# cvg/pixel-perfect-sfm

Measured on AMD Instinct MI355X. Metric: featuremetric residuals+Jacobians evaluated/sec (1M obs), higher is better.
Workload: dtype f32 horizontal / f64 vertical+normalisation on f16 patches; 1 GPU; BASELINE.json configs[2]: synthetic 200 cams / 200000 points / 1000000 obs featuremetric BA residual+Jacobian evaluation, 128-ch fp16 16x16 patches, SIMPLE_RADIAL, fused six-scalar Jacobian reduction; n_obs=1000000, channels=128, patch=16, obs_per_gpu=1000000, partition=none

## Files before the change

pixel-perfect-sfm_amd/csrc/pxr_ba_solve.hip:

```cpp
#include <hip/hip_runtime.h>

#include <algorithm>
#include <chrono>
#include <cmath>
#include <cstdlib>
#include <cstring>
#include <limits>
#include <thread>
#include <vector>

#include "pxr_ba_pcg.h"
#include "pxr_ba_solve.h"
#include "pxr_device.h"
#include "pxr_internal.h"

namespace pxr {


constexpr int JAC_THREADS = 128;

__global__ __launch_bounds__(JAC_THREADS) void k_jac(const SolveDev d, const double* __restrict__ rec,
                                                     pxr_loss loss, double* __restrict__ L, double* __restrict__ W) {
  extern __shared__ double jstage[];
  const int lane = threadIdx.x & 63, wave = threadIdx.x >> 6;
// ... 219 lines not shown
      double tr = 0.0;
      for (int x = 0; x < NP; ++x) tr += red[x];
      chunk_trace[blockIdx.x] = tr;
    }
  }
  if (sl == 0 && kpart) {
    kpart[(size_t)blockIdx.x * ne_max + e] = acc;
  } else if (sl == 0) {
    const int ra = col_index(d, img, cam, a);
    const double v = fixed ? __longlong_as_double(qacc) : acc;
    if (is_g) accum_flush(gc + ra, v, det_scale);
    else if (block_form) {
      double* Ub = U + (size_t)img * d.DC * d.DC;
      accum_flush(Ub + a * d.DC + b, v, det_scale);
      if (a != b) accum_flush(Ub + b * d.DC + a, v, det_scale);
    } else accum_flush(U + (size_t)ra * d.n_c + col_index(d, img, cam, b), v, det_scale);
  }
}

__global__ __launch_bounds__(256) void k_pinv(int64_t n_points, const int* __restrict__ pt_var,
                                              const double* __restrict__ V,
                                              const double* __restrict__ Vdiag0 ,
                                              double inv_radius, double* __restrict__ T,
                                              double* __restrict__ zero_ptr, int zero_n) {
  if (blockIdx.x == 0) for (int e = threadIdx.x; e < zero_n; e += blockDim.x) zero_ptr[e] = 0.0;
  const int64_t p = (int64_t)blockIdx.x * blockDim.x + threadIdx.x;
  if (p >= n_points) return;
  double* To = T + 6 * p;
  if (!pt_var[p]) { for (int j = 0; j < 6; ++j) To[j] = 0.0; return; }
  const double a00 = V[6 * p] + Vdiag0[3 * p] * inv_radius, a01 = V[6 * p + 1], a02 = V[6 * p + 2];
  const double a11 = V[6 * p + 3] + Vdiag0[3 * p + 1] * inv_radius, a12 = V[6 * p + 4];
  const double a22 = V[6 * p + 5] + Vdiag0[3 * p + 2] * inv_radius;
  const double c00 = a11 * a22 - a12 * a12, c01 = a02 * a12 - a01 * a22, c02 = a01 * a12 - a02 * a11;
  const double det = a00 * c00 + a01 * c01 + a02 * c02;
  const double id = 1.0 / det;
  To[0] = c00 * id; To[1] = c01 * id; To[2] = c02 * id;
  To[3] = (a00 * a22 - a02 * a02) * id; To[4] = (a01 * a02 - a00 * a12) * id;
  To[5] = (a00 * a11 - a01 * a01) * id;
}

struct Copy4 { const double* src[4]; double* dst[4]; int64_t n[4]; };
__global__ __launch_bounds__(256) void k_copy4(const Copy4 c) {
  const int64_t stride = (int64_t)gridDim.x * blockDim.x, t0 = (int64_t)blockIdx.x * blockDim.x + threadIdx.x;
#pragma unroll
  for (int a = 0; a < 4; ++a)
    for (int64_t e = t0; e < c.n[a]; e += stride) c.dst[a][e] = c.src[a][e];
}

__global__ __launch_bounds__(256) void k_schur(const SolveDev d, const int64_t* __restrict__ pt_ptr,
                                               const int64_t* __restrict__ pt_obs,
                                               const double* __restrict__ W, const double* __restrict__ T,
                                               const double* __restrict__ gp, double* __restrict__ S,
                                               double* __restrict__ rhs, double det_scale) {
  const int64_t tid = (int64_t)blockIdx.x * blockDim.x + threadIdx.x;
  const int64_t i = tid / d.DC;
  const int a = (int)(tid - i * d.DC);
  if (i >= d.v.n_obs) return;
  const int img = d.v.d_obs_image[i], cam = d.v.d_image_camera[img];
  const int dci = d.pose_dim[img] + d.intr_dim[cam];
  if (a >= dci) return;
  const int pt = d.v.d_obs_point[i];
  if (!d.pt_var[pt]) return;
  double y0, y1, y2;
  y_row(W, T, i, a, d.DC, pt, y0, y1, y2);
  const int r = col_index(d, img, cam, a);
  accum_add(rhs + (size_t)r * d.ldS, -(y0 * gp[3 * (size_t)pt] + y1 * gp[3 * (size_t)pt + 1] + y2 * gp[3 * (size_t)pt + 2]), det_scale);
  for (int64_t o = pt_ptr[pt]; o < pt_ptr[pt + 1]; ++o) {
    const int64_t j = pt_obs[o];
    const int imgj = d.v.d_obs_image[j], camj = d.v.d_image_camera[imgj];
// ... 82 lines not shown
            const int c = col[u];
            if (c >= 0 && c >= rrow[a])
              accum_add(acc + (size_t)a * CT + (c - c0), -(ya0 * mm[u][0] + ya1 * mm[u][1] + ya2 * mm[u][2]), det_scale);
          }
        }
      }
    }
    o = o_next; s = s_next;
  }
  __syncthreads();
  for (int e = threadIdx.x; e < dci * CT; e += blockDim.x) {
    const int a = e / CT, cl = e % CT;
    const double v = acc[(size_t)a * CT + cl];
    if (__double_as_longlong(v) != 0ll) accum_flush(S + (size_t)col_index(d, img, cam, a) * d.ldS + (c0 + cl), v, det_scale);
  }
  if (blockIdx.y == 0 && threadIdx.x < dci) {
    const double v = racc[threadIdx.x];
    if (__double_as_longlong(v) != 0ll) accum_flush(rhs + (size_t)col_index(d, img, cam, threadIdx.x) * d.ldS, v, det_scale);
  }
}

__global__ void k_copy_upper_add_diag(int n, const double* __restrict__ U, const double* __restrict__ damp,
                                      double inv_radius, const double* __restrict__ gc, double* __restrict__ S,
                                      int add_u, double det_scale) {
  const int64_t t = (int64_t)blockIdx.x * blockDim.x + threadIdx.x;
  const int ld = n + 1;
  if (t >= (int64_t)n * ld) return;
  const int r = (int)(t / ld), c = (int)(t % ld);
  double v = S[t];
  if (add_u) {
    v = (c < n && r <= c) ? U[(size_t)r * n + c] : 0.0;
  }
  else {
    if (det_scale != 0.0) v = (double)__double_as_longlong(v) / det_scale;
    if (r == c) v += damp[r] * inv_radius;
    if (c == n) v += gc[r];
  }
  S[t] = v;
}

__global__ void k_extract_diag(int n, const double* __restrict__ U, double* __restrict__ out) {
  const int i = blockIdx.x * blockDim.x + threadIdx.x;
  if (i < n) out[i] = U[(size_t)i * n + i];
}

__global__ void k_clamp(int64_t n, const double* __restrict__ in, double lo, double hi, double* __restrict__ out) {
  const int64_t i = (int64_t)blockIdx.x * blockDim.x + threadIdx.x;
  if (i < n) out[i] = fmin(fmax(in[i], lo), hi);
}

__global__ void k_point_diag(int64_t n_points, const double* __restrict__ V, double* __restrict__ out) {
  const int64_t p = (int64_t)blockIdx.x * blockDim.x + threadIdx.x;
  if (p >= n_points) return;
  out[3 * p] = V[6 * p]; out[3 * p + 1] = V[6 * p + 3]; out[3 * p + 2] = V[6 * p + 5];
}

__global__ void k_jacobi_scale(int64_t n, const double* __restrict__ diag, double* __restrict__ scale) {
  const int64_t i = (int64_t)blockIdx.x * blockDim.x + threadIdx.x;
  if (i < n) scale[i] = 1.0 / (1.0 + sqrt(diag[i]));
}

__global__ void k_axpy1(int n, const double* __restrict__ x, double* __restrict__ y) {
  const int i = blockIdx.x * blockDim.x + threadIdx.x;
  if (i < n) y[i] += x[i];
}

__global__ void k_fill(int64_t n, double v, double* __restrict__ out) {
  const int64_t i = (int64_t)blockIdx.x * blockDim.x + threadIdx.x;
  if (i < n) out[i] = v;
}

__global__ void k_finish_camera_step(int n, const double* __restrict__ x, const double* __restrict__ gc,
                                     const double* __restrict__ damp, double inv_radius,
                                     double* __restrict__ delta_c, double* __restrict__ scal_rep, long long* __restrict__ limb) {
  __shared__ long long lsh[PXR_LIMBS * 4];
  const int i = blockIdx.x * blockDim.x + threadIdx.x;
  double part = 0.0;
  if (i < n) {
    const double dl = -x[i];
    delta_c[i] = dl;
    part = dl * (damp[i] * inv_radius * dl - gc[i]);
  }
  if (limb) {
    Limbs l;
    if (i < n) l.add(part);
    limbs_block_add(l, limb + (8 + 0) * PXR_LIMBS, lsh);
    return;
  }
  for (int off = 32; off > 0; off >>= 1) part += __shfl_xor(part, off);
  if ((threadIdx.x & 63) == 0) atomicAdd(scal_rep + 0, part);
}

constexpr int BACKSUB_PPG = 8;
template <int G>
__global__ __launch_bounds__(256) void k_backsub(const SolveDev d, const int64_t* __restrict__ pt_ptr,
                                                 const int* __restrict__ pj, const int4* __restrict__ pcols,
                                                 const double* __restrict__ W, const double* __restrict__ T,
                                                 const double* __restrict__ gp, const double* __restrict__ delta_c,
                                                 const double* __restrict__ Vdiag0, double inv_radius,
                                                 double* __restrict__ delta_p, double* __restrict__ scal_sum, long long* __restrict__ limb) {
  __shared__ double red[256 / 64];
  __shared__ long long lsh[PXR_LIMBS * 4];
  const int lane_a = threadIdx.x % G;
  double part = 0.0;
  Limbs lpart;
  for (int rep = 0; rep < BACKSUB_PPG; ++rep) {
  const int64_t p = ((int64_t)blockIdx.x * BACKSUB_PPG + rep) * (256 / G) + threadIdx.x / G;
  const bool live = p < d.v.n_points;
  const bool var = live && d.pt_var[p];
  double v0 = 0.0, v1 = 0.0, v2 = 0.0;
  if (var) {
    const int64_t o_end = pt_ptr[p + 1];
    for (int64_t o = pt_ptr[p]; o < o_end; o += 4) {
      int4 ci[4];
      int jj[4];
#pragma unroll
      for (int u = 0; u < 4; ++u) { const int64_t idx = min(o + u, o_end - 1); ci[u] = pcols[idx]; jj[u] = pj[idx]; }
      double w[4][3], dcv[4];
      bool ok[4];
#pragma unroll
      for (int u = 0; u < 4; ++u) {
        ok[u] = o + u < o_end && lane_a < ci[u].y + ci[u].w;
        const double* Wi = W + ((size_t)jj[u] * d.DC + (ok[u] ? lane_a : 0)) * 3;
        w[u][0] = Wi[0]; w[u][1] = Wi[1]; w[u][2] = Wi[2];
        dcv[u] = delta_c[ok[u] ? (lane_a < ci[u].y ? ci[u].x + lane_a : ci[u].z + (lane_a - ci[u].y)) : 0];
      }
#pragma unroll
      for (int u = 0; u < 4; ++u)
        if (ok[u]) { v0 += w[u][0] * dcv[u]; v1 += w[u][1] * dcv[u]; v2 += w[u][2] * dcv[u]; }
    }
  }
#pragma unroll
  for (int off = G / 2; off > 0; off >>= 1) {
    v0 += __shfl_xor(v0, off); v1 += __shfl_xor(v1, off); v2 += __shfl_xor(v2, off);
  }
  if (live && lane_a == 0) {
    double dl[3] = {0, 0, 0};
    if (var) {
      v0 += gp[3 * p]; v1 += gp[3 * p + 1]; v2 += gp[3 * p + 2];
      const double* Tp = T + 6 * p;
      dl[0] = -(Tp[0] * v0 + Tp[1] * v1 + Tp[2] * v2);
      dl[1] = -(Tp[1] * v0 + Tp[3] * v1 + Tp[4] * v2);
      dl[2] = -(Tp[2] * v0 + Tp[4] * v1 + Tp[5] * v2);
      double pp = 0.0;
#pragma unroll
      for (int j = 0; j < 3; ++j) pp += dl[j] * (Vdiag0[3 * p + j] * inv_radius * dl[j] - gp[3 * p + j]);
      if (limb) lpart.add(pp); else part += pp;
    }
// ... 190 lines not shown
  }
}
__global__ __launch_bounds__(1024) void k_finish_and_stats(int n, int n_slots, double* __restrict__ gcd, double det_scale,
                                                            const long long* __restrict__ trace_limbs, double* __restrict__ out4) {
  __shared__ double smax[1024], ssum[1024], smin[1024];
  double mx = 0.0, sm = 0.0, mn = 0.0;
  for (int i = threadIdx.x; i < n_slots; i += 1024) {
    const double v = accum_value(gcd[i], det_scale);
    gcd[i] = v;
    if (i < n) { mx = fmax(mx, v); mn = fmin(mn, v); sm += v; }
  }
  smax[threadIdx.x] = mx; ssum[threadIdx.x] = sm; smin[threadIdx.x] = mn;
  __syncthreads();
  for (int off = 512; off > 0; off >>= 1) {
    if ((int)threadIdx.x < off) {
      smax[threadIdx.x] = fmax(smax[threadIdx.x], smax[threadIdx.x + off]);
      smin[threadIdx.x] = fmin(smin[threadIdx.x], smin[threadIdx.x + off]);
      ssum[threadIdx.x] += ssum[threadIdx.x + off];
    }
    __syncthreads();
  }
  if (threadIdx.x == 0) { out4[0] = smax[0]; out4[1] = ssum[0]; out4[2] = smin[0]; out4[3] = limb_value(trace_limbs); }
}
__global__ void k_i64_split(int64_t n, const long long* __restrict__ in, double* __restrict__ out) {
  const int64_t i = (int64_t)blockIdx.x * blockDim.x + threadIdx.x;
  if (i >= n) return;
  const long long v = in[i];
  out[2 * i] = (double)(int)(v >> 32);
  out[2 * i + 1] = (double)(unsigned)(v & 0xffffffffll);
}
__global__ void k_i64_join(int64_t n, const double* __restrict__ in, long long* __restrict__ out) {
  const int64_t i = (int64_t)blockIdx.x * blockDim.x + threadIdx.x;
  if (i >= n) return;
  const unsigned long long hi = (unsigned long long)(long long)in[2 * i], lo = (unsigned long long)(long long)in[2 * i + 1];
  out[i] = (long long)((hi << 32) + lo);
}

__global__ void k_zero(int64_t n, double* __restrict__ x) {
  const int64_t i = (int64_t)blockIdx.x * blockDim.x + threadIdx.x;
  if (i < n) x[i] = 0.0;
}

__global__ __launch_bounds__(256) void k_build_descriptors(int64_t n_obs, const int32_t* __restrict__ obs_image,
                                                           const int32_t* __restrict__ obs_point,
                                                           const int32_t* __restrict__ image_camera,
                                                           const int64_t* __restrict__ pt_obs, const int64_t* __restrict__ img_obs,
// ... 153 lines not shown
  *owned = true;
  if (hipMalloc(&p, b) != hipSuccess) { (void)hipGetLastError(); return nullptr; }
  return p;
}
template <typename T>
struct DevBuf {
  T* p = nullptr;
  size_t n = 0;
  bool owned = true;
  int alloc(size_t count) {
    n = count;
    p = static_cast<T*>(solve_scratch(sizeof(T) * (count ? count : 1), &owned));
    return p ? PXR_OK : set_error(PXR_ENOMEM, "hipMalloc(solver buffer): %zu bytes", sizeof(T) * count);
  }
  int upload(const std::vector<T>& h, hipStream_t s) {
    int rc = alloc(h.size());
    if (rc) return rc;
    if (!h.empty()) return hip_check(hipMemcpyAsync(p, h.data(), sizeof(T) * h.size(), hipMemcpyHostToDevice, s), "H2D");
    return PXR_OK;
  }
  ~DevBuf() { if (p && owned) (void)hipFree(p); }
};

int chol_factor_solve(hipStream_t st, double* a, int n, int* d_info, double* linv_ws, double* x_out, bool zero_info = true);
size_t chol_workspace_doubles(int n);
size_t inner_wave_stage_bytes(int64_t n_pts);

int launch_inner_iterations(pxr_ctx* ctx, pxr_arena* arena, const pxr_ba_view* view, const pxr_interp_cfg* cfg,
                            const pxr_loss* loss, const int64_t* d_pt_ptr, const int64_t* d_pt_obs,
                            const int* d_pt_var, double* d_cost_before, const InnerLists* lists, double* d_cost_per_point,
                            const GramCache* gram, bool gram_warm);
int make_inner_lists(pxr_ctx* ctx, const int64_t* h_pt_ptr, int64_t n_pts, void* h_wave_stage, size_t wave_stage_bytes, const pxr_ba_view* view, const int64_t* d_pt_ptr, const int64_t* d_pt_obs,
                     InnerLists* out);
void free_inner_lists(InnerLists* l);

static inline unsigned nblk(int64_t n, int b = 256) { return (unsigned)((n + b - 1) / b); }

#define RC(call) do { int _rc = (call); if (_rc != PXR_OK) return _rc; } while (0)
#define LAUNCH_CHECK(name) RC(hip_check(hipGetLastError(), name))

}

static int ba_solve_impl(pxr_ctx* ctx, pxr_arena* arena, const pxr_ba_view* view, const pxr_interp_cfg* cfg, const double* d_obs_xy,
                         const pxr_loss* loss, const uint8_t* h_pose_const, const uint8_t* h_tvec_const_mask,
                         const uint16_t* h_cam_const_mask, const uint8_t* h_point_const,
                         const pxr_lm_options* opt, pxr_allreduce_fn allreduce, void* ar_user,
                         pxr_lm_summary* sum) {
// ... 13 lines not shown
      on = !(e && e[0] == '0');
      a.base = static_cast<char*>(c->d_solve_arena); a.cap = c->solve_arena_bytes;
      if (on) g_solve_arena = &a;
    }
    ~ArenaScope() {
      g_solve_arena = nullptr;
      if (!on || a.wanted <= a.cap) return;
      (void)hipDeviceSynchronize();
      if (ctx->d_solve_arena) (void)hipFree(ctx->d_solve_arena);
      ctx->d_solve_arena = nullptr; ctx->solve_arena_bytes = 0;
      const size_t want = a.wanted + a.wanted / 16 + (1u << 20);
      if (hipMalloc(&ctx->d_solve_arena, want) == hipSuccess) ctx->solve_arena_bytes = want;
      else { (void)hipGetLastError(); ctx->d_solve_arena = nullptr; }
    }
  } arena_scope(ctx);
  const bool setup_verbose = std::getenv("PXR_VERBOSE") != nullptr;
  auto setup_mark = [&](const char* what) {
    if (setup_verbose)
      fprintf(stderr, "[pxr_ba_solve] setup: %-28s at %.2f ms\n", what,
              std::chrono::duration<double, std::milli>(std::chrono::steady_clock::now() - t_setup0).count());
  };
  const int64_t n_obs = view->n_obs, n_pts = view->n_points;
  const int n_img = view->n_images, n_cam = view->n_cameras;

  std::vector<int32_t> obs_image, obs_point, image_camera(n_img), cam_model(n_cam);
  std::vector<int64_t> img_cnt(n_img + 1, 0), pt_cnt;
  DevBuf<unsigned long long> d_cnt;
  DevBuf<int> d_flags;
  bool device_lists = n_img <= SORT_MAX_IMAGES && std::getenv("PXR_BA_SETUP_HOST") == nullptr;
  PXR_HIP(hipMemcpyAsync(image_camera.data(), view->d_image_camera, 4 * n_img, hipMemcpyDeviceToHost, st));
  PXR_HIP(hipMemcpyAsync(cam_model.data(), view->d_cam_model, 4 * n_cam, hipMemcpyDeviceToHost, st));
  setup_mark("camera tables read");
  if (device_lists) {
    int h_flags[2] = {0, 0};
    RC(d_cnt.alloc((size_t)n_img + 1 + (size_t)n_pts + 1 + 1)); RC(d_flags.alloc(2));
    setup_mark("counter buffers");
    PXR_HIP(hipMemsetAsync(d_cnt.p, 0, sizeof(unsigned long long) * d_cnt.n, st));
    PXR_HIP(hipMemsetAsync(d_flags.p, 0, sizeof(int) * 2, st));
    hipLaunchKernelGGL(k_count_indices, dim3((unsigned)((n_obs + COUNT_CHUNK - 1) / COUNT_CHUNK)), dim3(256), sizeof(unsigned int) * n_img, st, n_obs, view->d_obs_image,
                       view->d_obs_point, n_img, n_pts, d_cnt.p, d_cnt.p + n_img + 1, d_flags.p);
    static_assert(sizeof(unsigned long long) == sizeof(int64_t), "counter width");
    PXR_HIP(hipMemcpyAsync(img_cnt.data(), d_cnt.p, sizeof(int64_t) * (n_img + 1), hipMemcpyDeviceToHost, st));
    PXR_HIP(hipMemcpyAsync(h_flags, d_flags.p, sizeof(int) * 2, hipMemcpyDeviceToHost, st));
    PXR_HIP(hipStreamSynchronize(st));
    PXR_REQUIRE(h_flags[0] == 0, "pxr_ba_solve: an observation references an image / point out of range");
    if (h_flags[1]) {
// ... 303 lines not shown
  for (int c = 0; c < n_cam; ++c) gram_inner = gram_inner && cam_model[c] <= PXR_OPENCV;
  bool inner_cache = gram_inner && gram_eval_supported(arena, view) && !getenv("PXR_INNER_NO_CACHE");
  GramCache gram;
  if ((gram_cache || inner_cache) && gram_eval_prepare(ctx, arena, view, &gram) != PXR_OK) {
    gram_cache = false; inner_cache = false;
    (void)set_error(PXR_OK, "");
  }
  bool geom_ext = false;
  for (int c = 0; c < n_cam; ++c) geom_ext = geom_ext || cam_model[c] > PXR_OPENCV;
  setup_mark("Gram-matrix cache prepared");
  bool gram_warm = false;
  int n_evaluations = 0;
  bool cur_is_exact = true;
  auto evaluate = [&](const pxr_ba_view& v, double* rec) -> int {
    if (geom) RC(geom_eval(ctx, &v, d_obs_xy, rec, nullptr));
    else if (gram_cache && n_evaluations > 0) { RC(gram_evaluate(ctx, arena, &v, cfg, gram, rec)); gram_warm = true; }
    else RC(ba_eval_with_cost(ctx, arena, &v, cfg, 1, rec, nullptr, nullptr, nullptr, nullptr, nullptr));
    ++n_evaluations;
    hipLaunchKernelGGL(k_cost_limbs, dim3(1024), dim3(256), 0, st, (const double*)rec, n_obs, *loss, slimb.p + 0 * PXR_LIMBS);
    LAUNCH_CHECK("cost");
    return PXR_OK;
  };
  double lin_scale = 0.0;
  auto linearize = [&](const double* rec) -> int {
    hipLaunchKernelGGL(k_jac, dim3((unsigned)((n_obs + JAC_THREADS - 1) / JAC_THREADS)), dim3(JAC_THREADS),
                       sizeof(double) * (JAC_THREADS / 64) * 64 * (LS + 3 * DC + 1), st, dv, rec, *loss, L.p, W.p);
    hipLaunchKernelGGL(k_point, dim3(nblk(n_pts)), dim3(256), 0, st, dv, d_pt_ptr.p, d_pt_obs.p, L.p, V.p, gp.p);
    PXR_HIP(hipMemsetAsync(U.p, 0, sizeof(double) * U.n, st));
    PXR_HIP(hipMemsetAsync(gcd.p, 0, sizeof(double) * gcd.n, st));
    if (n_c > 0 && !chunks.empty()) {
      hipLaunchKernelGGL(k_img, dim3((unsigned)chunks.size()), dim3(256), sizeof(double) * ((size_t)IMG_BATCH * LS + 256), st, dv,
                         d_chunks.p, d_img_obs.p, L.p, U.p, gc, iterative ? 1 : 0, lin_scale, lin_scale != 0.0 ? chunk_trace.p : (double*)nullptr,
                         det_iter ? det_kpart.p : (double*)nullptr, det_ne_max);
      if (det_iter) {
        RC(pcg_blocks_from_partials(st, dv, d_kchunk_ptr.p, det_kpart.p, det_ne_max, U.p, det_gimg.p, d_col_ent_ptr.p, d_col_ent.p, diagU, gc));
        LAUNCH_CHECK("linearize kernels");
        RC(ar(gcd.p, 2 * (int64_t)nc1));
        return PXR_OK;
      }
      if (lin_scale != 0.0) {
        hipLaunchKernelGGL(k_diag_and_trace, dim3(1), dim3(1024), 0, st, n_c, (const double*)U.p, diagU, (const double*)chunk_trace.p, (int)chunks.size(),
                           reinterpret_cast<long long*>(gcd.p + 2 * nc1));
        RC(ar_i64(reinterpret_cast<long long*>(gcd.p), 2 * (int64_t)nc1 + PXR_LIMBS));
        hipLaunchKernelGGL(k_finish_and_stats, dim3(1), dim3(1024), 0, st, n_c, 2 * (int)nc1, gcd.p, lin_scale,
                           reinterpret_cast<const long long*>(gcd.p + 2 * nc1), lin_stats.p);
        LAUNCH_CHECK("linearize kernels");
        return PXR_OK;
      }
      if (iterative) RC(pcg_diag_from_blocks(st, dv, U.p, diagU));
      else hipLaunchKernelGGL(k_extract_diag, dim3(nblk(n_c)), dim3(256), 0, st, n_c, U.p, diagU);
    }
    LAUNCH_CHECK("linearize kernels");
    RC(ar(gcd.p, 2 * (int64_t)nc1));
    return PXR_OK;
  };
  auto lin_fits = [&](const double* stt, double md_made_for) {
    if (n_c == 0 || chunks.empty()) return true;
    const double mx = stt[0], sm = stt[1], mn = stt[2], tr = stt[3];
    if (!(std::isfinite(mx) && std::isfinite(sm) && std::isfinite(tr))) return false;
    if (mn < 0.0) return false;
    if (std::fabs(tr - sm) > std::ldexp(1.0, 61) / lin_scale) return false;
    return mx <= 8.0 * md_made_for;
  };
  bool lin_not_finite = false;
  auto linearize_checked = [&](const double* rec, double md_guess, double cost_now, bool refine = false) -> int {
    if (!det_fixed) return linearize(rec);
    for (int attempt = 0; attempt < 8; ++attempt) {
      lin_md = md_guess;
      lin_scale = det_scale_for(lin_md, cost_now);
      RC(linearize(rec));
      PXR_HIP(hipMemcpyAsync(h_lin_stats, lin_stats.p, sizeof(double) * 4, hipMemcpyDeviceToHost, st));
      PXR_HIP(hipStreamSynchronize(st));
      if (lin_fits(h_lin_stats, lin_md)) {
        if (refine && attempt == 0 && h_lin_stats[0] * 64.0 < md_guess) { md_guess = std::max(h_lin_stats[0], 1e-300); continue; }
        return PXR_OK;
      }
      if (!(std::isfinite(h_lin_stats[3]) && h_lin_stats[3] >= 0.0)) { lin_not_finite = true; return PXR_OK; }
      md_guess = std::max(h_lin_stats[3], 2.0 * md_guess);
    }
    return set_error(PXR_EINVAL, "pxr_ba_solve: the fixed-point grid of the deterministic mode could not be fitted");
  };
  auto refresh_damping = [&]() -> int {
    if (n_c > 0) hipLaunchKernelGGL(k_clamp, dim3(nblk(n_c)), dim3(256), 0, st, (int64_t)n_c, diagU, opt->min_lm_diagonal, opt->max_lm_diagonal, damp_c.p);
    hipLaunchKernelGGL(k_point_diag, dim3(nblk(n_pts)), dim3(256), 0, st, n_pts, V.p, Vd0.p);
    hipLaunchKernelGGL(k_clamp, dim3(nblk(n_pts * 3)), dim3(256), 0, st, n_pts * 3, Vd0.p, opt->min_lm_diagonal, opt->max_lm_diagonal, Vd0.p);
    LAUNCH_CHECK("damping kernels");
    return PXR_OK;
  };

  if (iterative) {
    pcg.st = st; pcg.dv = dv;
    pcg.chunks = d_schur_chunks.p; pcg.n_chunks = (int)schur_chunks.size(); pcg.so = d_so.p;
    pcg.pt_ptr = d_pt_ptr.p; pcg.part_obs = d_part_obs.p; pcg.obs_cols = d_obs_cols.p;
    pcg.W = W.p; pcg.T = T.p; pcg.gp = gp.p; pcg.gc = gc; pcg.damp_c = damp_c.p; pcg.Ublk = U.p;
    pcg.n_groups = (int)group_size.size(); pcg.col_group = d_col_group.p; pcg.group_size = d_group_size.p;
    pcg.group_cols = d_group_cols.p;
    pcg.u = pcg_u.p; pcg.Mloc = pcg_mloc.p; pcg.Gm = pcg_g.p;
    pcg.x = xsol.p; pcg.r = pcg_vec.p; pcg.p = pcg_vec.p + nc1; pcg.q = pcg_vec.p + 2 * nc1; pcg.z = pcg_vec.p + 3 * nc1;
    pcg.b = pcg_vec.p + 4 * nc1; pcg.cgs = pcg_scal.p; pcg.cg_part = pcg_scal.p + 16; pcg.d_fail = d_info;
    pcg.det = det_iter;
    if (det_iter) {
      pcg.chunk_ptr = d_schunk_ptr.p; pcg.col_ent_ptr = d_col_ent_ptr.p; pcg.col_ent = d_col_ent.p;
      pcg.wpart = det_wpart.p; pcg.mpart = det_mpart.p;
    }
  }
// ... 122 lines not shown
        return 1;
      rc = h[0] > 0.0 ? 1 : (h[1] > 0.0 ? 2 : 0);
    }
    return rc;
  };
  auto user_stop = [&](int rc) {
    if (rc == 1) { sum->termination = PXR_TERM_FAILURE; return true; }
    if (rc == 2) { sum->termination = PXR_TERM_CONVERGENCE; return true; }
    return false;
  };
  if (user_stop(notify(0, false, false, cost, 0.0, 0.0, radius, 0.0))) {
    sum->final_cost = cost; sum->final_radius = radius;
    sum->total_ms = std::chrono::duration<double, std::milli>(std::chrono::steady_clock::now() - t_loop0).count();
    return PXR_OK;
  }

  while (true) {
    if (sum->iterations >= opt->max_iterations) { sum->termination = PXR_TERM_NO_CONVERGENCE; break; }
    if (radius < opt->min_radius) { sum->termination = PXR_TERM_CONVERGENCE; break; }
    ++sum->iterations;
    phase(7);
    if (!reuse_diag) RC(refresh_damping());
    const double inv_radius = 1.0 / radius;
    hipLaunchKernelGGL(k_pinv, dim3(nblk(n_pts)), dim3(256), 0, st, n_pts, d_pt_var.p, V.p, Vd0.p, inv_radius, T.p, scal.p, 16 + 16 * PXR_LIMBS + 1);
    if (n_pts == 0) RC(zero_scalars());
    bool ok = true;
    double inexact_correction = 0.0;
    if (n_c > 0 && iterative) {
      PcgResult pr;
      RC(pcg_solve(pcg, inv_radius, opt, ar_fn, &pr));
      phase(2);
      sum->linear_iterations += pr.iterations;
      if (!pr.ok) ok = false;
      inexact_correction = 0.5 * pr.x_dot_r;
      PXR_HIP(hipMemsetAsync(d_info, 0, sizeof(int), st));
      hipLaunchKernelGGL(k_finish_camera_step, dim3(nblk(n_c)), dim3(256), 0, st, n_c, xsol.p, gc, damp_c.p, inv_radius, delta_c.p, scal_rep, limb_arg);
      RC(from_rank0(delta_c.p, n_c));
    } else if (n_c > 0) {
      const double schur_scale = det_fixed ? lin_scale : 0.0;
      hipLaunchKernelGGL(k_copy_upper_add_diag, dim3(nblk((int64_t)n_c * ldS)), dim3(256), 0, st, n_c, U.p, (const double*)nullptr, 0.0, (const double*)nullptr, S.p, 1, schur_scale);
      if (use_lds_schur) {
#define SCHUR_LAUNCH(GG)                                                                                              \
  hipLaunchKernelGGL(k_schur_lds<GG>, dim3((unsigned)schur_chunks.size(), (unsigned)n_ctiles), dim3(1024), schur_shmem, st, dv, \
                     d_schur_chunks.p, d_so.p, d_part_obs.p, d_obs_cols.p, W.p, T.p, gp.p, CT, S.p, rhs, schur_scale)
        if (DC <= 8) SCHUR_LAUNCH(8); else if (DC <= 16) SCHUR_LAUNCH(16); else SCHUR_LAUNCH(32);
#undef SCHUR_LAUNCH
      } else {
        hipLaunchKernelGGL(k_schur, dim3(nblk(n_obs * DC)), dim3(256), 0, st, dv, d_pt_ptr.p, d_pt_obs.p, W.p, T.p, gp.p, S.p, rhs, schur_scale);
      }
      LAUNCH_CHECK("schur kernels");
      phase(0);
      if (multi) {
        hipLaunchKernelGGL(k_pack_upper, dim3((unsigned)n_c), dim3(256), 0, st, n_c, S.p, S_packed.p);
        if (schur_scale != 0.0) RC(ar_i64(reinterpret_cast<long long*>(S_packed.p), packed_doubles));
        else RC(ar(S_packed.p, packed_doubles));
        hipLaunchKernelGGL(k_unpack_upper, dim3((unsigned)n_c), dim3(256), 0, st, n_c, S_packed.p, S.p);
        LAUNCH_CHECK("pack / unpack of the reduced camera system");
      }
      phase(1);
      hipLaunchKernelGGL(k_copy_upper_add_diag, dim3(nblk((int64_t)n_c * ldS)), dim3(256), 0, st, n_c, U.p, damp_c.p, inv_radius, gc, S.p, 0, schur_scale);
      RC(chol_factor_solve(st, S.p, n_c, d_info, linv.p, xsol.p, false));
      phase(2);
      hipLaunchKernelGGL(k_finish_camera_step, dim3(nblk(n_c)), dim3(256), 0, st, n_c, xsol.p, gc, damp_c.p, inv_radius, delta_c.p, scal_rep, limb_arg);
      RC(from_rank0(delta_c.p, n_c));
    }
    phase(3);
    double model_cost_change = 0, cand_cost = 0, step_norm = 0, x_norm = 0;
    if (ok) {
#define BACKSUB_LAUNCH(GG)                                                                                                          \
  hipLaunchKernelGGL(k_backsub<GG>, dim3(nblk((n_pts * GG + BACKSUB_PPG - 1) / BACKSUB_PPG)), dim3(256), 0, st, dv, d_pt_ptr.p, d_part_obs.p, d_obs_cols.p, W.p, T.p, gp.p, \
                     delta_c.p, Vd0.p, inv_radius, delta_p.p, scal_sum, limb_arg)
      if (DC <= 8) BACKSUB_LAUNCH(8); else if (DC <= 16) BACKSUB_LAUNCH(16); else BACKSUB_LAUNCH(32);
#undef BACKSUB_LAUNCH
      ParamPtrs out{q1.p, t1.p, k1.p, X1.p};
      const int64_t upd_blocks = nblk(((int64_t)n_img + n_cam + n_pts + UPDATE_IPT - 1) / UPDATE_IPT);
      hipLaunchKernelGGL(k_update, dim3((unsigned)upd_blocks), dim3(256), 0, st, dv, delta_c.p, delta_p.p, out, scal_rep, scal_sum, limb_arg);
      LAUNCH_CHECK("step kernels");
      const bool do_inner = inner_enabled;
      if (do_inner) {
        PXR_HIP(hipMemsetAsync(det_part.p, 0, sizeof(double) * (size_t)n_pts, st));
        if (geom) RC(launch_inner_geom(ctx, &cand_view, d_obs_xy, loss, d_pt_ptr.p, d_pt_obs.p, d_pt_var.p, scal_sum + 4, det_part.p, geom_ext));
        else {
          RC(launch_inner_iterations(ctx, arena, &cand_view, cfg, loss, d_pt_ptr.p, d_pt_obs.p, d_pt_var.p, scal_sum + 4, gram_inner ? &inner_lists.l : nullptr,
                                     det_part.p, (gram_cache || inner_cache) ? &gram : nullptr, gram_warm));
          gram_warm = true;
        }
        hipLaunchKernelGGL(k_limb_accumulate, dim3(256), dim3(256), 0, st, (const double*)det_part.p, n_pts, slimb.p + 4 * PXR_LIMBS);
        PXR_HIP(hipMemsetAsync(scal_sum + 2, 0, sizeof(double), st));
        PXR_HIP(hipMemsetAsync(slimb.p + 2 * PXR_LIMBS, 0, sizeof(long long) * PXR_LIMBS, st));
        hipLaunchKernelGGL(k_point_step_norm, dim3(nblk(n_pts)), dim3(256), 0, st, n_pts, d_pt_var.p, cur_X, X1.p, scal_sum + 2,
                           det ? slimb.p + 2 * PXR_LIMBS : (long long*)nullptr);
        LAUNCH_CHECK("inner iteration kernels");
      }
      phase(4);
      RC(evaluate(cand_view, rec_cand));
      RC(read_scal(hs));
      const int h_info = *h_info_word;
      if (det_fixed && !lin_fits(h_lin_stats, lin_md)) {
        RC(linearize_checked(rec_cur, std::max(h_lin_stats[3], 2.0 * lin_md), cost));
        if (lin_not_finite) { sum->termination = PXR_TERM_FAILURE; break; }
        --sum->iterations;
        continue;
      }
// ... 20 lines not shown
      if (!(gram_cache && cur_is_exact && n_evaluations > 1)) return PXR_OK;
      double h2[16];
      RC(zero_scalars());
      RC(evaluate(dv.v, rec_cur));
      RC(read_scal(h2));
      if (std::isfinite(h2[0])) cost = h2[0];
      cur_is_exact = false;
      return PXR_OK;
    };
    if (!ok) {
      if (++invalid >= opt->max_consecutive_invalid_steps) { sum->termination = PXR_TERM_FAILURE; break; }
      radius *= 0.5; reuse_diag = true;
      if (user_stop(notify(sum->iterations, false, false, cost, 0.0, 0.0, radius, step_norm))) break;
      continue;
    }
    invalid = 0;
    if (step_norm <= opt->parameter_tolerance * (x_norm + opt->parameter_tolerance)) { sum->termination = PXR_TERM_CONVERGENCE; break; }
    const double cost_change = cost - cand_cost;
    if (std::fabs(cost_change) <= opt->function_tolerance * cost) { sum->termination = PXR_TERM_CONVERGENCE; break; }
    const double rel = cost_change / model_cost_change;
    if (inner_useful || rel > opt->min_relative_decrease) {
      {
        Copy4 c4{{q1.p, t1.p, k1.p, X1.p}, {cur_q, cur_t, cur_k, cur_X},
                 {(int64_t)4 * n_img, (int64_t)3 * n_img, (int64_t)PXR_KPAD * n_cam, (int64_t)3 * n_pts}};
        hipLaunchKernelGGL(k_copy4, dim3((unsigned)std::min<int64_t>(1024, nblk(3 * n_pts + 1))), dim3(256), 0, st, c4);
      }
      std::swap(rec_cur, rec_cand);
      cost = cand_cost;
      cur_is_exact = false;
      if (det_fixed) { lin_md = std::max(h_lin_stats[0], 1e-300); lin_scale = det_scale_for(lin_md, cost); }
      RC(linearize(rec_cur));
      phase(6);
      ++sum->num_successful;
      const double tmp = 2.0 * rel - 1.0;
      radius = radius / std::max(1.0 / 3.0, 1.0 - tmp * tmp * tmp);
      radius = std::min(opt->max_radius, radius);
      decrease_factor = 2.0; reuse_diag = false;
      if (opt->gradient_tolerance > 0.0) {
        bool below = false;
        RC(gradient_below_tolerance(&below));
        if (below) { sum->termination = PXR_TERM_CONVERGENCE; break; }
      }
      if (user_stop(notify(sum->iterations, true, true, cost, cost_change, rel, radius, step_norm))) break;
    } else {
      RC(reevaluate_current());
      radius = radius / decrease_factor; decrease_factor *= 2.0; reuse_diag = true;
      if (user_stop(notify(sum->iterations, true, false, cost, cost_change, rel, radius, step_norm))) break;
    }
  }
  PXR_HIP(hipStreamSynchronize(st));
  if (phase_timing)
    fprintf(stderr, "[pxr_ba_solve] phase ms over %d iterations: schur-build %.2f allreduce %.2f potrf %.2f potrs %.2f "
            "backsub+update %.2f eval+cost %.2f linearize %.2f other %.2f\n", sum->iterations, ph_ms[0], ph_ms[1],
            ph_ms[2], ph_ms[3], ph_ms[4], ph_ms[5], ph_ms[6], ph_ms[7]);
// ... 25 lines not shown
```

pixel-perfect-sfm_amd/csrc/pxr_chol.hip:

```cpp
#include <hip/hip_runtime.h>

#include <cstdlib>

#include "pxr_chol_core.h"
#include "pxr_internal.h"

namespace pxr {

constexpr int CNB = 64;
typedef double mfma_d4 __attribute__((ext_vector_type(4)));
constexpr int SPAD = CNB + 8;

struct PanelLds {
  cholcore::FactorLds f;
  double U[CNB][CNB + 16 * cholcore::ROW_WAVES];
  double H[3][4][CNB];
};
struct UpdateLds {
  double Pi[CNB][SPAD];
  double Pj[CNB][SPAD];
};
constexpr size_t kStepLdsNeed = sizeof(PanelLds) > sizeof(UpdateLds) ? sizeof(PanelLds) : sizeof(UpdateLds);
constexpr size_t kStepLds = kStepLdsNeed > 96 * 1024 ? kStepLdsNeed : 96 * 1024;

// ... 208 lines not shown
    if (tid < CNB) z[tid] -= part[0][tid] + part[1][tid] + part[2][tid] + part[3][tid];
  }
  __syncthreads();
  const double* Li = linv + (size_t)c * CNB * CNB;
  double s = 0.0;
#pragma unroll
  for (int q = 0; q < 16; ++q) {
    const int r = sl * 16 + q;
    s = fma(Li[r * CNB + j], z[r], s);
  }
  part[sl][j] = s;
  __syncthreads();
  if (tid < nbc) __hip_atomic_store(&x_out[c0 + tid], part[0][tid] + part[1][tid] + part[2][tid] + part[3][tid],
                                    __ATOMIC_RELAXED, __HIP_MEMORY_SCOPE_AGENT);
  __syncthreads();
  if (tid == 0) {
    __threadfence();
    __hip_atomic_store(&flags[c], 1, __ATOMIC_RELEASE, __HIP_MEMORY_SCOPE_AGENT);
  }
}

size_t chol_workspace_doubles(int n) { return (size_t)(2 * ((n + CNB - 1) / CNB) + 1) * CNB * CNB; }

int chol_factor_solve(hipStream_t st, double* a, int n, int* d_info, double* linv_ws, double* x_out, bool zero_info) {
  const int lda = n + 1, n_rows = n + 1;
  const int nblk = (n + CNB - 1) / CNB;
  if (int rc = hip_check(hipFuncSetAttribute((const void*)k_chol_step, hipFuncAttributeMaxDynamicSharedMemorySize, (int)kStepLds), "LDS size")) return rc;
  if (zero_info) if (int rc = hip_check(hipMemsetAsync(d_info, 0, sizeof(int), st), "memset info")) return rc;
  const int rows_per_wg = 16 * cholcore::ROW_WAVES;
  int* flags = reinterpret_cast<int*>(linv_ws + (size_t)nblk * CNB * CNB);
  const size_t spare_ints = sizeof(double) * CNB * CNB / sizeof(int);
  if ((size_t)nblk > spare_ints) return set_error(PXR_EINVAL, "chol_factor_solve: n = %d too large", n);
  const bool one_launch_fits = (size_t)nblk * (1 + kDoneStride) <= spare_ints;
  const bool step_launches = std::getenv("PXR_CHOL_ONE_LAUNCH") == nullptr || !one_launch_fits;
  if (int rc = hip_check(hipMemsetAsync(flags, 0, sizeof(int) * (step_launches ? (size_t)nblk : (size_t)nblk * (1 + kDoneStride)), st), "memset flags")) return rc;
  long long total_wgs = 0;
  for (int s = 0, k = 0; k < n; ++s, k += CNB) {
    const int nb = (n - k < CNB) ? n - k : CNB;
    const int rem = n_rows - k - nb;
    const int n_panel = (CNB + rem + rows_per_wg - 1) / rows_per_wg;
    const int T = (n_rows - k + CNB - 1) / CNB;
    const int n_update = s > 0 ? T * (T - 1) / 2 : 0;
    total_wgs += n_panel + n_update;
    if (step_launches)
      hipLaunchKernelGGL(k_chol_step, dim3(n_panel + n_update), dim3(512), kStepLds, st, a, n_rows, n, lda, s, n_panel, d_info, linv_ws,
                         linv_ws + (size_t)(nblk + 1) * CNB * CNB);
  }
  if (!step_launches) {
    if (total_wgs > 0x7fffffffll) return set_error(PXR_EINVAL, "chol_factor_solve: n = %d too large for one launch", n);
    if (int rc = hip_check(hipFuncSetAttribute((const void*)k_chol_all, hipFuncAttributeMaxDynamicSharedMemorySize, (int)kStepLds), "LDS size")) return rc;
    hipLaunchKernelGGL(k_chol_all, dim3((unsigned)total_wgs), dim3(512), kStepLds, st, a, n_rows, n, lda, d_info, linv_ws,
                       linv_ws + (size_t)(nblk + 1) * CNB * CNB, flags + nblk);
  }
  hipLaunchKernelGGL(k_chol_backsolve, dim3(nblk), dim3(256), 0, st, a, n, lda, linv_ws, x_out, flags, nblk);
  return hip_check(hipGetLastError(), "cholesky launch");
}

__global__ void k_aug_pack(int n, const double* __restrict__ a, const double* __restrict__ b, double* __restrict__ aug) {
// ... 7 lines not shown
}
__global__ void k_aug_unpack(int n, const double* __restrict__ aug, const double* __restrict__ ldiag, double* __restrict__ a) {
  const int64_t t = (int64_t)blockIdx.x * blockDim.x + threadIdx.x;
  if (t >= (int64_t)n * n) return;
  const int r = (int)(t / n), c = (int)(t % n);
  if (r <= c) a[t] = (r / CNB == c / CNB) ? ldiag[(size_t)(r / CNB) * CNB * CNB + (c % CNB) + (r % CNB) * CNB] : aug[(size_t)r * (n + 1) + c];
}

}

extern "C" int pxr_dense_spd_solve(pxr_ctx* ctx, double* d_a, int n, double* d_b, int* h_info) {
  using namespace pxr;
  PXR_REQUIRE(ctx && d_a && d_b && h_info && n > 0, "pxr_dense_spd_solve: invalid argument");
  PXR_HIP(hipSetDevice(ctx->device));
  hipStream_t st = ctx->stream;
  double *aug = nullptr, *linv = nullptr;
  const size_t na = (size_t)(n + 1) * (n + 1), nl = chol_workspace_doubles(n);
  if (hipMalloc((void**)&aug, sizeof(double) * na) != hipSuccess || hipMalloc((void**)&linv, sizeof(double) * nl) != hipSuccess) {
    (void)hipFree(aug); (void)hipFree(linv);
    return set_error(PXR_ENOMEM, "pxr_dense_spd_solve: workspace allocation failed");
  }
  int* d_info = reinterpret_cast<int*>(ctx->d_scratch);
  hipLaunchKernelGGL(k_aug_pack, dim3((unsigned)((na + 255) / 256)), dim3(256), 0, st, n, d_a, d_b, aug);
  int rc = chol_factor_solve(st, aug, n, d_info, linv, d_b, true);
  if (!rc) {
    hipLaunchKernelGGL(k_aug_unpack, dim3((unsigned)(((size_t)n * n + 255) / 256)), dim3(256), 0, st, n, aug,
                       linv + (size_t)((n + CNB - 1) / CNB + 1) * CNB * CNB, d_a);
    rc = hip_check(hipMemcpyAsync(h_info, d_info, sizeof(int), hipMemcpyDeviceToHost, st), "D2H info");
  }
  if (!rc) rc = hip_check(hipStreamSynchronize(st), "sync");
  (void)hipFree(aug); (void)hipFree(linv);
  return rc;
}
```

Measured before the change: 1.416 billion residual_blocks/s.

## Fuse small LM-loop kernels and memsets into neighbouring kernels

```diff
diff --git a/pixel-perfect-sfm_amd/csrc/pxr_ba_solve.hip b/pixel-perfect-sfm_amd/csrc/pxr_ba_solve.hip
--- a/pixel-perfect-sfm_amd/csrc/pxr_ba_solve.hip
+++ b/pixel-perfect-sfm_amd/csrc/pxr_ba_solve.hip
@@ -265,10 +265,11 @@
                                               const double* __restrict__ V,
                                               const double* __restrict__ Vdiag0 ,
                                               double inv_radius, double* __restrict__ T,
-                                              double* __restrict__ zero_ptr, int zero_n) {
+                                              double* __restrict__ zero_ptr, int zero_n, double* __restrict__ zero_pts) {
   if (blockIdx.x == 0) for (int e = threadIdx.x; e < zero_n; e += blockDim.x) zero_ptr[e] = 0.0;
   const int64_t p = (int64_t)blockIdx.x * blockDim.x + threadIdx.x;
   if (p >= n_points) return;
+  if (zero_pts) zero_pts[p] = 0.0;
   double* To = T + 6 * p;
   if (!pt_var[p]) { for (int j = 0; j < 6; ++j) To[j] = 0.0; return; }
   const double a00 = V[6 * p] + Vdiag0[3 * p] * inv_radius, a01 = V[6 * p + 1], a02 = V[6 * p + 2];
@@ -282,12 +283,15 @@
   To[5] = (a00 * a11 - a01 * a01) * id;
 }
 
-struct Copy4 { const double* src[4]; double* dst[4]; int64_t n[4]; };
+struct Copy4 { const double* src[4]; double* dst[4]; int64_t n[4]; double* z[2]; int64_t zn[2]; };
 __global__ __launch_bounds__(256) void k_copy4(const Copy4 c) {
   const int64_t stride = (int64_t)gridDim.x * blockDim.x, t0 = (int64_t)blockIdx.x * blockDim.x + threadIdx.x;
 #pragma unroll
   for (int a = 0; a < 4; ++a)
     for (int64_t e = t0; e < c.n[a]; e += stride) c.dst[a][e] = c.src[a][e];
+#pragma unroll
+  for (int a = 0; a < 2; ++a)
+    for (int64_t e = t0; e < c.zn[a]; e += stride) c.z[a][e] = 0.0;
 }
 
 __global__ __launch_bounds__(256) void k_schur(const SolveDev d, const int64_t* __restrict__ pt_ptr,
@@ -416,8 +420,9 @@
 
 __global__ void k_copy_upper_add_diag(int n, const double* __restrict__ U, const double* __restrict__ damp,
                                       double inv_radius, const double* __restrict__ gc, double* __restrict__ S,
-                                      int add_u, double det_scale) {
+                                      int add_u, double det_scale, int* __restrict__ zero_flags, int zero_n) {
   const int64_t t = (int64_t)blockIdx.x * blockDim.x + threadIdx.x;
+  if (t < zero_n) zero_flags[t] = 0;
   const int ld = n + 1;
   if (t >= (int64_t)n * ld) return;
   const int r = (int)(t / ld), c = (int)(t % ld);
@@ -447,6 +452,17 @@
   const int64_t p = (int64_t)blockIdx.x * blockDim.x + threadIdx.x;
   if (p >= n_points) return;
   out[3 * p] = V[6 * p]; out[3 * p + 1] = V[6 * p + 3]; out[3 * p + 2] = V[6 * p + 5];
+}
+
+__global__ void k_refresh_damping(int n_c, const double* __restrict__ diagU, int64_t n_points, const double* __restrict__ V,
+                                  double lo, double hi, double* __restrict__ damp_c, double* __restrict__ Vd0) {
+  const int64_t i = (int64_t)blockIdx.x * blockDim.x + threadIdx.x;
+  if (i < n_c) damp_c[i] = fmin(fmax(diagU[i], lo), hi);
+  if (i < n_points) {
+    Vd0[3 * i] = fmin(fmax(V[6 * i], lo), hi);
+    Vd0[3 * i + 1] = fmin(fmax(V[6 * i + 3], lo), hi);
+    Vd0[3 * i + 2] = fmin(fmax(V[6 * i + 5], lo), hi);
+  }
 }
 
 __global__ void k_jacobi_scale(int64_t n, const double* __restrict__ diag, double* __restrict__ scale) {
@@ -486,18 +502,39 @@
 }
 
 constexpr int BACKSUB_PPG = 8;
+struct BacksubFused {
+  const double* cam_x; const double* cam_gc; const double* cam_damp; double* cam_delta_c; double* cam_scal_rep;
+};
 template <int G>
 __global__ __launch_bounds__(256) void k_backsub(const SolveDev d, const int64_t* __restrict__ pt_ptr,
                                                  const int* __restrict__ pj, const int4* __restrict__ pcols,
                                                  const double* __restrict__ W, const double* __restrict__ T,
                                                  const double* __restrict__ gp, const double* __restrict__ delta_c,
                                                  const double* __restrict__ Vdiag0, double inv_radius,
-                                                 double* __restrict__ delta_p, double* __restrict__ scal_sum, long long* __restrict__ limb) {
+                                                 double* __restrict__ delta_p, double* __restrict__ scal_sum, long long* __restrict__ limb,
+                                                 const BacksubFused f) {
   __shared__ double red[256 / 64];
   __shared__ long long lsh[PXR_LIMBS * 4];
   const int lane_a = threadIdx.x % G;
   double part = 0.0;
   Limbs lpart;
+  const bool cam_fused = f.cam_x != nullptr;
+  const double* __restrict__ dc_in = cam_fused ? f.cam_x : delta_c;
+  if (cam_fused && blockIdx.x == 0) {
+    double cpart = 0.0;
+    Limbs lc;
+    for (int i = threadIdx.x; i < d.n_c; i += 256) {
+      const double dl = -f.cam_x[i];
+      f.cam_delta_c[i] = dl;
+      const double pc = dl * (f.cam_damp[i] * inv_radius * dl - f.cam_gc[i]);
+      if (limb) lc.add(pc); else cpart += pc;
+    }
+    if (limb) { limbs_block_add(lc, limb + (8 + 0) * PXR_LIMBS, lsh); __syncthreads(); }
+    else {
+      cpart = wave_sum(cpart);
+      if ((threadIdx.x & 63) == 0) atomicAdd(f.cam_scal_rep + 0, cpart);
+    }
+  }
   for (int rep = 0; rep < BACKSUB_PPG; ++rep) {
   const int64_t p = ((int64_t)blockIdx.x * BACKSUB_PPG + rep) * (256 / G) + threadIdx.x / G;
   const bool live = p < d.v.n_points;
@@ -517,7 +554,8 @@
         ok[u] = o + u < o_end && lane_a < ci[u].y + ci[u].w;
         const double* Wi = W + ((size_t)jj[u] * d.DC + (ok[u] ? lane_a : 0)) * 3;
         w[u][0] = Wi[0]; w[u][1] = Wi[1]; w[u][2] = Wi[2];
-        dcv[u] = delta_c[ok[u] ? (lane_a < ci[u].y ? ci[u].x + lane_a : ci[u].z + (lane_a - ci[u].y)) : 0];
+        dcv[u] = dc_in[ok[u] ? (lane_a < ci[u].y ? ci[u].x + lane_a : ci[u].z + (lane_a - ci[u].y)) : 0];
+        if (cam_fused) dcv[u] = -dcv[u];
       }
 #pragma unroll
       for (int u = 0; u < 4; ++u)
@@ -754,6 +792,35 @@
   }
   if (threadIdx.x == 0) { out4[0] = smax[0]; out4[1] = ssum[0]; out4[2] = smin[0]; out4[3] = limb_value(trace_limbs); }
 }
+__global__ __launch_bounds__(1024) void k_diag_trace_finish(int n, const double* __restrict__ U, int n_slots, double* __restrict__ gcd,
+                                                             const double* __restrict__ chunk_trace, int n_chunks, long long* __restrict__ trace_out,
+                                                             double det_scale, double* __restrict__ out4) {
+  __shared__ double sh[1024], smax[1024], ssum[1024], smin[1024];
+  double acc = 0.0;
+  for (int i = threadIdx.x; i < n_chunks; i += 1024) acc += chunk_trace[i];
+  double mx = 0.0, sm = 0.0, mn = 0.0;
+  for (int i = threadIdx.x; i < n_slots; i += 1024) {
+    const double v = accum_value(i < n ? U[(size_t)i * n + i] : gcd[i], det_scale);
+    gcd[i] = v;
+    if (i < n) { mx = fmax(mx, v); mn = fmin(mn, v); sm += v; }
+  }
+  sh[threadIdx.x] = acc; smax[threadIdx.x] = mx; ssum[threadIdx.x] = sm; smin[threadIdx.x] = mn;
+  __syncthreads();
+  for (int off = 512; off > 0; off >>= 1) {
+    if ((int)threadIdx.x < off) {
+      sh[threadIdx.x] += sh[threadIdx.x + off];
+      smax[threadIdx.x] = fmax(smax[threadIdx.x], smax[threadIdx.x + off]);
+      smin[threadIdx.x] = fmin(smin[threadIdx.x], smin[threadIdx.x + off]);
+      ssum[threadIdx.x] += ssum[threadIdx.x + off];
+    }
+    __syncthreads();
+  }
+  if (threadIdx.x == 0) {
+    Limbs l; l.add(sh[0]);
+    for (int k = 0; k < PXR_LIMBS; ++k) trace_out[k] = l.q[k];
+    out4[0] = smax[0]; out4[1] = ssum[0]; out4[2] = smin[0]; out4[3] = limb_value(l.q);
+  }
+}
 __global__ void k_i64_split(int64_t n, const long long* __restrict__ in, double* __restrict__ out) {
   const int64_t i = (int64_t)blockIdx.x * blockDim.x + threadIdx.x;
   if (i >= n) return;
@@ -953,7 +1020,8 @@
   ~DevBuf() { if (p && owned) (void)hipFree(p); }
 };
 
-int chol_factor_solve(hipStream_t st, double* a, int n, int* d_info, double* linv_ws, double* x_out, bool zero_info = true);
+int chol_factor_solve(hipStream_t st, double* a, int n, int* d_info, double* linv_ws, double* x_out, bool zero_info = true, bool zero_flags = true);
+int* chol_step_flags(double* linv_ws, int n, int* count);
 size_t chol_workspace_doubles(int n);
 size_t inner_wave_stage_bytes(int64_t n_pts);
 
@@ -1013,6 +1081,8 @@
   };
   const int64_t n_obs = view->n_obs, n_pts = view->n_points;
   const int n_img = view->n_images, n_cam = view->n_cameras;
+  const char* const unfused_env = std::getenv("PXR_LM_UNFUSED");
+  const bool lm_fused = !(unfused_env && unfused_env[0] != '\0' && unfused_env[0] != '0');
 
   std::vector<int32_t> obs_image, obs_point, image_camera(n_img), cam_model(n_cam);
   std::vector<int64_t> img_cnt(n_img + 1, 0), pt_cnt;
@@ -1362,12 +1432,14 @@
     return PXR_OK;
   };
   double lin_scale = 0.0;
-  auto linearize = [&](const double* rec) -> int {
+  auto linearize = [&](const double* rec, bool cleared = false) -> int {
     hipLaunchKernelGGL(k_jac, dim3((unsigned)((n_obs + JAC_THREADS - 1) / JAC_THREADS)), dim3(JAC_THREADS),
                        sizeof(double) * (JAC_THREADS / 64) * 64 * (LS + 3 * DC + 1), st, dv, rec, *loss, L.p, W.p);
     hipLaunchKernelGGL(k_point, dim3(nblk(n_pts)), dim3(256), 0, st, dv, d_pt_ptr.p, d_pt_obs.p, L.p, V.p, gp.p);
-    PXR_HIP(hipMemsetAsync(U.p, 0, sizeof(double) * U.n, st));
-    PXR_HIP(hipMemsetAsync(gcd.p, 0, sizeof(double) * gcd.n, st));
+    if (!cleared) {
+      PXR_HIP(hipMemsetAsync(U.p, 0, sizeof(double) * U.n, st));
+      PXR_HIP(hipMemsetAsync(gcd.p, 0, sizeof(double) * gcd.n, st));
+    }
     if (n_c > 0 && !chunks.empty()) {
       hipLaunchKernelGGL(k_img, dim3((unsigned)chunks.size()), dim3(256), sizeof(double) * ((size_t)IMG_BATCH * LS + 256), st, dv,
                          d_chunks.p, d_img_obs.p, L.p, U.p, gc, iterative ? 1 : 0, lin_scale, lin_scale != 0.0 ? chunk_trace.p : (double*)nullptr,
@@ -1376,6 +1448,12 @@
         RC(pcg_blocks_from_partials(st, dv, d_kchunk_ptr.p, det_kpart.p, det_ne_max, U.p, det_gimg.p, d_col_ent_ptr.p, d_col_ent.p, diagU, gc));
         LAUNCH_CHECK("linearize kernels");
         RC(ar(gcd.p, 2 * (int64_t)nc1));
+        return PXR_OK;
+      }
+      if (lin_scale != 0.0 && lm_fused && !multi) {
+        hipLaunchKernelGGL(k_diag_trace_finish, dim3(1), dim3(1024), 0, st, n_c, (const double*)U.p, 2 * (int)nc1, gcd.p, (const double*)chunk_trace.p,
+                           (int)chunks.size(), reinterpret_cast<long long*>(gcd.p + 2 * nc1), lin_scale, lin_stats.p);
+        LAUNCH_CHECK("linearize kernels");
         return PXR_OK;
       }
       if (lin_scale != 0.0) {
@@ -1421,6 +1499,12 @@
     return set_error(PXR_EINVAL, "pxr_ba_solve: the fixed-point grid of the deterministic mode could not be fitted");
   };
   auto refresh_damping = [&]() -> int {
+    if (lm_fused) {
+      hipLaunchKernelGGL(k_refresh_damping, dim3(nblk(std::max<int64_t>(n_c, n_pts))), dim3(256), 0, st, n_c, (const double*)diagU, n_pts, (const double*)V.p,
+                         opt->min_lm_diagonal, opt->max_lm_diagonal, damp_c.p, Vd0.p);
+      LAUNCH_CHECK("damping kernel");
+      return PXR_OK;
+    }
     if (n_c > 0) hipLaunchKernelGGL(k_clamp, dim3(nblk(n_c)), dim3(256), 0, st, (int64_t)n_c, diagU, opt->min_lm_diagonal, opt->max_lm_diagonal, damp_c.p);
     hipLaunchKernelGGL(k_point_diag, dim3(nblk(n_pts)), dim3(256), 0, st, n_pts, V.p, Vd0.p);
     hipLaunchKernelGGL(k_clamp, dim3(nblk(n_pts * 3)), dim3(256), 0, st, n_pts * 3, Vd0.p, opt->min_lm_diagonal, opt->max_lm_diagonal, Vd0.p);
@@ -1589,10 +1673,12 @@
     phase(7);
     if (!reuse_diag) RC(refresh_damping());
     const double inv_radius = 1.0 / radius;
-    hipLaunchKernelGGL(k_pinv, dim3(nblk(n_pts)), dim3(256), 0, st, n_pts, d_pt_var.p, V.p, Vd0.p, inv_radius, T.p, scal.p, 16 + 16 * PXR_LIMBS + 1);
+    hipLaunchKernelGGL(k_pinv, dim3(nblk(n_pts)), dim3(256), 0, st, n_pts, d_pt_var.p, V.p, Vd0.p, inv_radius, T.p, scal.p, 16 + 16 * PXR_LIMBS + 1,
+                       (lm_fused && inner_enabled) ? det_part.p : (double*)nullptr);
     if (n_pts == 0) RC(zero_scalars());
     bool ok = true;
     double inexact_correction = 0.0;
+    const bool fuse_cam = lm_fused && n_c > 0 && n_pts > 0 && !bcast;
     if (n_c > 0 && iterative) {
       PcgResult pr;
       RC(pcg_solve(pcg, inv_radius, opt, ar_fn, &pr));
@@ -1601,11 +1687,12 @@
       if (!pr.ok) ok = false;
       inexact_correction = 0.5 * pr.x_dot_r;
       PXR_HIP(hipMemsetAsync(d_info, 0, sizeof(int), st));
-      hipLaunchKernelGGL(k_finish_camera_step, dim3(nblk(n_c)), dim3(256), 0, st, n_c, xsol.p, gc, damp_c.p, inv_radius, delta_c.p, scal_rep, limb_arg);
+      if (!(fuse_cam && ok)) hipLaunchKernelGGL(k_finish_camera_step, dim3(nblk(n_c)), dim3(256), 0, st, n_c, xsol.p, gc, damp_c.p, inv_radius, delta_c.p, scal_rep, limb_arg);
       RC(from_rank0(delta_c.p, n_c));
     } else if (n_c > 0) {
       const double schur_scale = det_fixed ? lin_scale : 0.0;
-      hipLaunchKernelGGL(k_copy_upper_add_diag, dim3(nblk((int64_t)n_c * ldS)), dim3(256), 0, st, n_c, U.p, (const double*)nullptr, 0.0, (const double*)nullptr, S.p, 1, schur_scale);
+      hipLaunchKernelGGL(k_copy_upper_add_diag, dim3(nblk((int64_t)n_c * ldS)), dim3(256), 0, st, n_c, U.p, (const double*)nullptr, 0.0, (const double*)nullptr, S.p, 1, schur_scale,
+                         (int*)nullptr, 0);
       if (use_lds_schur) {
 #define SCHUR_LAUNCH(GG)                                                                                              \
   hipLaunchKernelGGL(k_schur_lds<GG>, dim3((unsigned)schur_chunks.size(), (unsigned)n_ctiles), dim3(1024), schur_shmem, st, dv, \
@@ -1625,10 +1712,13 @@
         LAUNCH_CHECK("pack / unpack of the reduced camera system");
       }
       phase(1);
-      hipLaunchKernelGGL(k_copy_upper_add_diag, dim3(nblk((int64_t)n_c * ldS)), dim3(256), 0, st, n_c, U.p, damp_c.p, inv_radius, gc, S.p, 0, schur_scale);
-      RC(chol_factor_solve(st, S.p, n_c, d_info, linv.p, xsol.p, false));
+      int n_chol_flags = 0;
+      int* const chol_flags = lm_fused ? chol_step_flags(linv.p, n_c, &n_chol_flags) : nullptr;
+      hipLaunchKernelGGL(k_copy_upper_add_diag, dim3(nblk((int64_t)n_c * ldS)), dim3(256), 0, st, n_c, U.p, damp_c.p, inv_radius, gc, S.p, 0, schur_scale,
+                         chol_flags, n_chol_flags);
+      RC(chol_factor_solve(st, S.p, n_c, d_info, linv.p, xsol.p, false, chol_flags == nullptr));
       phase(2);
-      hipLaunchKernelGGL(k_finish_camera_step, dim3(nblk(n_c)), dim3(256), 0, st, n_c, xsol.p, gc, damp_c.p, inv_radius, delta_c.p, scal_rep, limb_arg);
+      if (!fuse_cam) hipLaunchKernelGGL(k_finish_camera_step, dim3(nblk(n_c)), dim3(256), 0, st, n_c, xsol.p, gc, damp_c.p, inv_radius, delta_c.p, scal_rep, limb_arg);
       RC(from_rank0(delta_c.p, n_c));
     }
     phase(3);
@@ -1636,7 +1726,9 @@
     if (ok) {
 #define BACKSUB_LAUNCH(GG)                                                                                                          \
   hipLaunchKernelGGL(k_backsub<GG>, dim3(nblk((n_pts * GG + BACKSUB_PPG - 1) / BACKSUB_PPG)), dim3(256), 0, st, dv, d_pt_ptr.p, d_part_obs.p, d_obs_cols.p, W.p, T.p, gp.p, \
-                     delta_c.p, Vd0.p, inv_radius, delta_p.p, scal_sum, limb_arg)
+                     delta_c.p, Vd0.p, inv_radius, delta_p.p, scal_sum, limb_arg, bf)
+      BacksubFused bf{nullptr, nullptr, nullptr, nullptr, nullptr};
+      if (fuse_cam) { bf.cam_x = xsol.p; bf.cam_gc = gc; bf.cam_damp = damp_c.p; bf.cam_delta_c = delta_c.p; bf.cam_scal_rep = scal_rep; }
       if (DC <= 8) BACKSUB_LAUNCH(8); else if (DC <= 16) BACKSUB_LAUNCH(16); else BACKSUB_LAUNCH(32);
 #undef BACKSUB_LAUNCH
       ParamPtrs out{q1.p, t1.p, k1.p, X1.p};
@@ -1645,7 +1737,7 @@
       LAUNCH_CHECK("step kernels");
       const bool do_inner = inner_enabled;
       if (do_inner) {
-        PXR_HIP(hipMemsetAsync(det_part.p, 0, sizeof(double) * (size_t)n_pts, st));
+        if (!lm_fused) PXR_HIP(hipMemsetAsync(det_part.p, 0, sizeof(double) * (size_t)n_pts, st));
         if (geom) RC(launch_inner_geom(ctx, &cand_view, d_obs_xy, loss, d_pt_ptr.p, d_pt_obs.p, d_pt_var.p, scal_sum + 4, det_part.p, geom_ext));
         else {
           RC(launch_inner_iterations(ctx, arena, &cand_view, cfg, loss, d_pt_ptr.p, d_pt_obs.p, d_pt_var.p, scal_sum + 4, gram_inner ? &inner_lists.l : nullptr,
@@ -1712,14 +1804,15 @@
     if (inner_useful || rel > opt->min_relative_decrease) {
       {
         Copy4 c4{{q1.p, t1.p, k1.p, X1.p}, {cur_q, cur_t, cur_k, cur_X},
-                 {(int64_t)4 * n_img, (int64_t)3 * n_img, (int64_t)PXR_KPAD * n_cam, (int64_t)3 * n_pts}};
-        hipLaunchKernelGGL(k_copy4, dim3((unsigned)std::min<int64_t>(1024, nblk(3 * n_pts + 1))), dim3(256), 0, st, c4);
+                 {(int64_t)4 * n_img, (int64_t)3 * n_img, (int64_t)PXR_KPAD * n_cam, (int64_t)3 * n_pts},
+                 {U.p, gcd.p}, {lm_fused ? (int64_t)U.n : 0, lm_fused ? (int64_t)gcd.n : 0}};
+        hipLaunchKernelGGL(k_copy4, dim3((unsigned)std::min<int64_t>(1024, nblk(std::max<int64_t>(3 * n_pts + 1, lm_fused ? (int64_t)U.n / 8 : 0)))), dim3(256), 0, st, c4);
       }
       std::swap(rec_cur, rec_cand);
       cost = cand_cost;
       cur_is_exact = false;
       if (det_fixed) { lin_md = std::max(h_lin_stats[0], 1e-300); lin_scale = det_scale_for(lin_md, cost); }
-      RC(linearize(rec_cur));
+      RC(linearize(rec_cur, lm_fused));
       phase(6);
       ++sum->num_successful;
       const double tmp = 2.0 * rel - 1.0;
diff --git a/pixel-perfect-sfm_amd/csrc/pxr_chol.hip b/pixel-perfect-sfm_amd/csrc/pxr_chol.hip
--- a/pixel-perfect-sfm_amd/csrc/pxr_chol.hip
+++ b/pixel-perfect-sfm_amd/csrc/pxr_chol.hip
@@ -254,7 +254,15 @@
 
 size_t chol_workspace_doubles(int n) { return (size_t)(2 * ((n + CNB - 1) / CNB) + 1) * CNB * CNB; }
 
-int chol_factor_solve(hipStream_t st, double* a, int n, int* d_info, double* linv_ws, double* x_out, bool zero_info) {
+int* chol_step_flags(double* linv_ws, int n, int* count) {
+  const int nblk = (n + CNB - 1) / CNB;
+  *count = 0;
+  if (std::getenv("PXR_CHOL_ONE_LAUNCH") != nullptr || (size_t)nblk > sizeof(double) * CNB * CNB / sizeof(int)) return nullptr;
+  *count = nblk;
+  return reinterpret_cast<int*>(linv_ws + (size_t)nblk * CNB * CNB);
+}
+
+int chol_factor_solve(hipStream_t st, double* a, int n, int* d_info, double* linv_ws, double* x_out, bool zero_info, bool zero_flags) {
   const int lda = n + 1, n_rows = n + 1;
   const int nblk = (n + CNB - 1) / CNB;
   if (int rc = hip_check(hipFuncSetAttribute((const void*)k_chol_step, hipFuncAttributeMaxDynamicSharedMemorySize, (int)kStepLds), "LDS size")) return rc;
@@ -265,7 +273,8 @@
   if ((size_t)nblk > spare_ints) return set_error(PXR_EINVAL, "chol_factor_solve: n = %d too large", n);
   const bool one_launch_fits = (size_t)nblk * (1 + kDoneStride) <= spare_ints;
   const bool step_launches = std::getenv("PXR_CHOL_ONE_LAUNCH") == nullptr || !one_launch_fits;
-  if (int rc = hip_check(hipMemsetAsync(flags, 0, sizeof(int) * (step_launches ? (size_t)nblk : (size_t)nblk * (1 + kDoneStride)), st), "memset flags")) return rc;
+  if (zero_flags || !step_launches)
+    if (int rc = hip_check(hipMemsetAsync(flags, 0, sizeof(int) * (step_launches ? (size_t)nblk : (size_t)nblk * (1 + kDoneStride)), st), "memset flags")) return rc;
   long long total_wgs = 0;
   for (int s = 0, k = 0; k < n; ++s, k += CNB) {
     const int nb = (n - k < CNB) ? n - k : CNB;
@@ -319,7 +328,7 @@
   }
   int* d_info = reinterpret_cast<int*>(ctx->d_scratch);
   hipLaunchKernelGGL(k_aug_pack, dim3((unsigned)((na + 255) / 256)), dim3(256), 0, st, n, d_a, d_b, aug);
-  int rc = chol_factor_solve(st, aug, n, d_info, linv, d_b, true);
+  int rc = chol_factor_solve(st, aug, n, d_info, linv, d_b, true, true);
   if (!rc) {
     hipLaunchKernelGGL(k_aug_unpack, dim3((unsigned)(((size_t)n * n + 255) / 256)), dim3(256), 0, st, n, aug,
                        linv + (size_t)((n + CNB - 1) / CNB + 1) * CNB * CNB, d_a);
```

Measured after the change: 1.416 billion residual_blocks/s (median of 2 runs). No clear change (-0.0%).
